# Urist-McDeveloper/nbody

Measured on AMD Instinct MI355X. Metric: particle-pair interactions/sec at N=2^20, higher is better.
Workload: dtype f32

## Files before the change

nbody_amd/csrc/kernels.h:

```cpp
#pragma once

#include <hip/hip_runtime.h>
#include <stdint.h>

namespace nb {

enum : uint32_t {
    STEP_ACC_IN = 1u,
    STEP_NO_FINALIZE = 2u,
};

enum : int {
    VARIANT_LDS = 0,
    VARIANT_SMEM = 1,
};

struct StepParams {
    const float2 *src_pos;
    const float *src_gm;
    uint32_t src_begin[2];
    uint32_t src_end[2];
    const float2 *pos_in;
    float2 *pos_out;
    float2 *vel;
    float2 *acc;
    const float *radius;
    uint32_t n_recv;
    uint32_t recv_split;
    uint32_t recv_gap;
    float2 *mirror;
    uint32_t n_mirror;
    const float *dt;
    uint32_t flags;
    float2 *parts;
    uint32_t split;
    uint32_t *tickets;
    uint32_t unit;
};

__host__ __device__ inline StepParams plain_step(const float2 *src_pos, const float *src_gm, uint32_t n_src, const float2 *pos_in,
                                                 float2 *pos_out, float2 *vel, float2 *acc, const float *radius, uint32_t n_recv,
                                                 const float *dt, uint32_t unit) {
    return StepParams{.src_pos = src_pos, .src_gm = src_gm, .src_begin = {0, 0}, .src_end = {n_src, 0}, .pos_in = pos_in,
                      .pos_out = pos_out, .vel = vel, .acc = acc, .radius = radius, .n_recv = n_recv, .recv_split = n_recv,
                      .dt = dt, .split = 1, .unit = unit};
}

struct ChainParams {
    float2 *pos;
    float2 *vel;
    float2 *acc;
// ... 34 lines not shown
};

struct RaggedParams {
    BatchParams b;
    const uint32_t *n_len;
    const uint32_t *members;
};

struct RaggedTraceParams {
    BatchTraceParams t;
    const uint32_t *n_len;
    const uint32_t *members;
};

constexpr int MAX_SPLIT = 16;

struct LaunchShape;

const void *step_kernel_fn(LaunchShape s);
const void *step_kernel_fused_fn(LaunchShape s);
const void *finish_kernel_fn();

void launch_chain(hipStream_t st, const ChainParams &p);

const void *batch_lane_split_fn(int w, int lanes);
void launch_batch_chain(hipStream_t st, const BatchParams &p, uint32_t count);
void launch_batch_trace_chain(hipStream_t st, const BatchTraceParams &p);

const void *ragged_lane_split_fn(int w, int lanes);
void launch_ragged_chain(hipStream_t st, const RaggedParams &p, uint32_t members);
void launch_ragged_trace_chain(hipStream_t st, const RaggedTraceParams &p, uint32_t members);

}
```

nbody_amd/csrc/kernels.hip:

```cpp
#include "kernels.h"
#include "diag_common.h"
#include "interaction_asm.h"
#include "launch_shape.h"

#include <hip/hip_runtime.h>

namespace nb {
namespace {

constexpr int WAVE = 64;
constexpr int CHUNK = 64;
constexpr int CLOSE_EVERY = 4;

typedef float v16f __attribute__((ext_vector_type(16)));
typedef float v8f __attribute__((ext_vector_type(8)));
typedef float v4f __attribute__((ext_vector_type(4)));

typedef float f2v __attribute__((ext_vector_type(2)));

template <int K>
struct Receivers {
    f2v p[K];
    float r[K];
    f2v a[K];
    f2v s[K];
    f2v c[K];
    __device__ __forceinline__ void clear() {
#pragma unroll
        for (int k = 0; k < K; k++) a[k] = s[k] = c[k] = f2v{0.0f, 0.0f};
    }
    __device__ __forceinline__ void close_chunk() {
#pragma unroll
        for (int k = 0; k < K; k++) {
            const f2v y = a[k] - c[k];
            const f2v t = s[k] + y;
            const f2v cn = (t - s[k]) - y;
            const bool lx = a[k].x != 0.0f, ly = a[k].y != 0.0f;
            const bool fx = __builtin_fabsf(t.x) < __builtin_inff(), fy = __builtin_fabsf(t.y) < __builtin_inff();
            c[k].x = lx ? (fx ? cn.x : 0.0f) : c[k].x;
            c[k].y = ly ? (fy ? cn.y : 0.0f) : c[k].y;
            s[k].x = lx ? t.x : s[k].x;
            s[k].y = ly ? t.y : s[k].y;
            a[k] = f2v{0.0f, 0.0f};
        }
    }
};


#define NB_INTERACT2(SRC)                                                                                                       \
    asm(NB_INTERACTION2_ASM                                                                                                     \
        : [ax0] "+v"(R.a[0].x), [ay0] "+v"(R.a[0].y), [ax1] "+v"(R.a[1].x), [ay1] "+v"(R.a[1].y)                                \
        : [sx] SRC(sxy.x), [sy] SRC(sxy.y), [g] SRC(sg), [px0] "v"(R.p[0].x), [py0] "v"(R.p[0].y), [r0] "v"(R.r[0]),            \
          [px1] "v"(R.p[1].x), [py1] "v"(R.p[1].y), [r1] "v"(R.r[1])                                                            \
        : NB_CLOBBERS2)
#define NB_INTERACT1(SRC)                                                                                                       \
    asm(NB_INTERACTION_ASM                                                                                                      \
        : [ax] "+v"(R.a[k].x), [ay] "+v"(R.a[k].y)                                                                              \
        : [sx] SRC(sxy.x), [sy] SRC(sxy.y), [g] SRC(sg), [px] "v"(R.p[k].x), [py] "v"(R.p[k].y), [r] "v"(R.r[k])                \
        : NB_CLOBBERS)
template <int K, bool SRC_IN_SGPR>
// ... 107 lines not shown
    const uint32_t logical = blockIdx.x * blockDim.x + threadIdx.x;
    if (logical >= p.n_recv) return;
    const uint32_t i = receiver_slot(p, logical);
    float2 part[MAX_SPLIT];
#pragma unroll
    for (uint32_t s = 0; s < (uint32_t)MAX_SPLIT; s++)
        part[s] = p.parts[(size_t)(s < p.split ? s : p.split - 1) * p.n_recv + logical];
    const float2 a0 = p.acc[i];
    const float2 v0 = p.vel[i];
    const float2 q0 = p.pos_in[i];
    const float dt = *p.dt;
    float sx = 0.0f, sy = 0.0f;
#pragma unroll
    for (uint32_t s = 0; s < (uint32_t)MAX_SPLIT; s++) add_part(sx, sy, part[s], s < p.split);
    finish_loaded(p, i, make_float2(sx, sy), a0, v0, q0, dt);
}

template <int K, int W, int VARIANT, bool FUSED = false>
__global__ __launch_bounds__(WAVE *W, 8) void step_kernel(const StepParams p) {
    const uint32_t tid = threadIdx.x;
    const uint32_t lane = tid & (WAVE - 1);
    const uint32_t wid = __builtin_amdgcn_readfirstlane(tid >> 6);
    const uint32_t tile_x = blockIdx.x, part_y = blockIdx.y;

    __shared__ __attribute__((aligned(16))) float tile[VARIANT == VARIANT_LDS ? W : 1][2][3 * CHUNK];
    __shared__ float2 partial[W > 1 ? W : 1][W > 1 ? WAVE * K : 1];

    const float dt = *p.dt;

    const uint32_t recv_base = tile_x * (WAVE * K);
// ... 36 lines not shown
            if (c + 1 < c_hi) fetch(c + 1);
            __builtin_amdgcn_fence(__ATOMIC_RELEASE, "wavefront");
            __builtin_amdgcn_wave_barrier();
            __builtin_amdgcn_fence(__ATOMIC_ACQUIRE, "wavefront");
            for (int jj = 0; jj < CHUNK; jj += 4) {
                const v8f P = *reinterpret_cast<const v8f *>(&T[buf][2 * jj]);
                const v4f G = *reinterpret_cast<const v4f *>(&T[buf][2 * CHUNK + jj]);
#pragma unroll
                for (int u = 0; u < 4; u++) interact<K, false>(R, f2v{P[2 * u], P[2 * u + 1]}, G[u]);
            }
            if (((c - c_lo) & (CLOSE_EVERY - 1)) == CLOSE_EVERY - 1) R.close_chunk();
            buf ^= 1;
        }
        if ((c_hi - c_lo) & (CLOSE_EVERY - 1)) R.close_chunk();
    } else {
#pragma unroll
        for (int range = 0; range < 2; range++) {
            const uint32_t r_lo = range == 0 ? 0u : n0;
            const uint32_t r_hi = range == 0 ? n0 : total;
            const uint32_t a = max(v_lo, r_lo), b = min(v_hi, r_hi);
            if (a >= b) continue;
            uint32_t j = p.src_begin[range] + (a - r_lo);
            const uint32_t j_end = p.src_begin[range] + (b - r_lo);
            const float *sp = reinterpret_cast<const float *>(p.src_pos), *sg = p.src_gm;
            const uint32_t groups = (j_end - j) / 8;
            const uint32_t g0 = (a - v_lo) / 8;
            if (groups > 0) {
                const uint32_t j_last = j + (groups - 1) * 8;
                v16f PA = src_load<v16f>(sp + 2 * (size_t)j);
                v8f GA = src_load<v8f>(sg + j);
                uint32_t g = 0;
                while (g + 2 <= groups) {
                    const uint32_t to_close = (8u * CLOSE_EVERY - ((g0 + g) & (8u * CLOSE_EVERY - 1))) / 2;
                    const uint32_t pairs = min(to_close, (groups - g) / 2);
                    for (uint32_t i = 0; i < pairs; i++) {
                        asm("" : "+s"(j) : "s"(PA), "s"(GA));
                        const v16f PB = src_load<v16f>(sp + 2 * (size_t)(j + 8));
                        const v8f GB = src_load<v8f>(sg + j + 8);
                        __builtin_amdgcn_sched_barrier(0);
                        interact8<K, true>(R, PA, GA);
                        __builtin_amdgcn_sched_barrier(0);
                        j = min(j + 16, j_last);
                        asm("" : "+s"(j) : "s"(PB), "s"(GB));
                        PA = src_load<v16f>(sp + 2 * (size_t)j);
                        GA = src_load<v8f>(sg + j);
                        __builtin_amdgcn_sched_barrier(0);
                        interact8<K, true>(R, PB, GB);
                    }
                    g += 2 * pairs;
                    if (pairs == to_close) R.close_chunk();
                }
                if (g < groups) interact8<K, true>(R, PA, GA);
                j = j_last + 8;
            }
            for (; j < j_end; j++) interact<K, true>(R, f2v{sp[2 * (size_t)j], sp[2 * (size_t)j + 1]}, sg[j]);
        }
        if ((v_hi - v_lo) & (CHUNK * CLOSE_EVERY - 1)) R.close_chunk();
    }

    auto finish = [&](uint32_t logical, float sx, float sy) {
        if (p.split > 1) {
            if (logical < p.n_recv) {
                float2 *slot = &p.parts[(size_t)part_y * p.n_recv + logical];
                if constexpr (FUSED) {
                    const uint64_t bits = (uint64_t)__float_as_uint(sx) | ((uint64_t)__float_as_uint(sy) << 32);
                    __hip_atomic_store(reinterpret_cast<uint64_t *>(slot), bits, __ATOMIC_RELAXED, __HIP_MEMORY_SCOPE_AGENT);
                } else {
                    *slot = make_float2(sx, sy);
                }
            }
        } else {
            finish_receiver(p, logical, sx, sy, dt);
        }
    };
// ... 32 lines not shown
                    for (uint32_t s = 0; s < (uint32_t)MAX_SPLIT; s++) {
                        const uint64_t bits = __hip_atomic_load(reinterpret_cast<const uint64_t *>(&p.parts[(size_t)(s < p.split ? s : p.split - 1) * p.n_recv + logical]),
                                                                __ATOMIC_RELAXED, __HIP_MEMORY_SCOPE_AGENT);
                        part[s] = make_float2(__uint_as_float((uint32_t)bits), __uint_as_float((uint32_t)(bits >> 32)));
                    }
                    const uint32_t i = receiver_slot(p, logical);
                    const float2 a0 = p.acc[i], v0 = p.vel[i], q0 = p.pos_in[i];
                    float sx = 0.0f, sy = 0.0f;
#pragma unroll
                    for (uint32_t s = 0; s < (uint32_t)MAX_SPLIT; s++) add_part(sx, sy, part[s], s < p.split);
                    finish_loaded(p, i, make_float2(sx, sy), a0, v0, q0, dt);
                }
            }
        }
    }
}

template <int W, int H>
__device__ __forceinline__ void lane_split_body(const StepParams &p) {
    constexpr uint32_t R = WAVE / H;
    constexpr uint32_t V = W * H;
    constexpr uint32_t T = 2 * WAVE * W;
    extern __shared__ __attribute__((aligned(16))) unsigned char lds_raw[];
    float2 *sxy = reinterpret_cast<float2 *>(lds_raw);
    float *sgm = reinterpret_cast<float *>(sxy + T);
    float2 *partial = reinterpret_cast<float2 *>(sgm + T);
    const uint32_t n0 = p.src_end[0] - p.src_begin[0];
    const uint32_t ntiles = (n0 + T - 1) / T;

    const uint32_t tid = threadIdx.x;
// ... 371 lines not shown

}

const void *step_kernel_fn(LaunchShape s) {
    if (s.lanes > 1) return pick_lane_split(s.w, s.lanes);
    return s.variant == VARIANT_SMEM ? pick<VARIANT_SMEM>(s.k, s.w) : pick<VARIANT_LDS>(s.k, s.w);
}

const void *step_kernel_fused_fn(LaunchShape s) {
    if (s.lanes > 1 || s.variant != VARIANT_SMEM) return nullptr;
    return pick_fused(s.k, s.w);
}

const void *finish_kernel_fn() { return reinterpret_cast<const void *>(&finish_kernel); }

const void *batch_lane_split_fn(int a, int b) {
    NB_CASE(batch_lane_split_kernel, 8, 8) NB_CASE(batch_lane_split_kernel, 16, 4)
    return nullptr;
}

const void *ragged_lane_split_fn(int a, int b) {
    NB_CASE(ragged_lane_split_kernel, 8, 8) NB_CASE(ragged_lane_split_kernel, 16, 4)
    return nullptr;
}
#undef NB_CASE

void launch_chain(hipStream_t st, const ChainParams &p) {
    hipLaunchKernelGGL(chain_kernel, dim3(1), dim3(1024), 0, st, p);
}

// ... 18 lines not shown
```

nbody_amd/csrc/launch_shape.h:

```cpp
#pragma once

#include "kernels.h"

namespace nb {

constexpr uint32_t BATCH_MAX_RECV = 3000;

struct LaunchShape {
    int k = 0;
    int w = 0;
    int variant = VARIANT_SMEM;
    int split = 0;
    int unit = 0;
    int lanes = 0;
};

inline bool operator==(const LaunchShape &a, const LaunchShape &b) {
    return a.k == b.k && a.w == b.w && a.variant == b.variant && a.split == b.split && a.unit == b.unit && a.lanes == b.lanes;
}

inline bool shape_on_auto(const LaunchShape &want) { return want == LaunchShape{}; }

constexpr uint32_t LANE_SPLIT_MAX_SRC = 1u << 18;

int lane_split_rule(uint32_t n_recv, uint32_t n_src, int *w);

LaunchShape choose_shape(LaunchShape want, uint32_t n_recv, uint32_t n_src, int compute_units);

bool fused_finish_rule(uint32_t n_recv, uint32_t n_src);

dim3 step_grid(LaunchShape s, uint32_t n_recv);
dim3 step_block(LaunchShape s);
size_t step_lds_bytes(LaunchShape s, uint32_t n_src);
dim3 finish_grid(uint32_t n_recv);
dim3 finish_block();

uint32_t chain_tiles(uint32_t n_recv);

int batch_lane_shape(uint32_t n_recv, int *w);

}
```

nbody_amd/csrc/launch_shape.hip:

```cpp
#include "launch_shape.h"

namespace nb {
namespace {

constexpr int WAVE = 64;
constexpr int CHUNK = 64;

double small_launch_cost_us(uint32_t n_recv, uint32_t n_src, int k, int w, int sp, int unit, int cus) {
    constexpr double LAT = 1.575, THR = 0.7545, K1 = 0.987, K1A = 0.178, A = 0.179, MIX = 0.874;
    constexpr double FINISH = 2.08, W4 = 1.035, UFIX = 0.15, BASE = 2.27;
    const uint32_t granules = (n_src + unit - 1) / unit;
    const uint64_t groups = ((uint64_t)n_recv + WAVE * k - 1) / (WAVE * k) * (uint64_t)sp;
    const uint64_t capacity = (uint64_t)cus * (32 / w);
    const uint64_t full = groups / capacity, left = groups % capacity;
    const uint32_t part_granules = (granules + sp - 1) / sp;
    const uint32_t wave_granules = (part_granules + w - 1) / w;
    const double units = (double)k * (wave_granules ? wave_granules : 1) * (double)unit / (double)CHUNK + UFIX;
    auto chunk_time = [&](double occ) {
        const double f = k == 1 ? K1 + K1A * (8.0 - occ) / 8.0 : 1.0;
        const double busy = occ * THR * f * (1.0 + A * (8.0 - occ) / 8.0);
        return LAT > busy ? LAT : busy;
    };
    double t = (double)full * units * chunk_time(8.0);
    if (left) {
// ... 116 lines not shown
uint32_t chain_tiles(uint32_t n_recv) {
    for (uint32_t t = 1; t <= 4; t *= 2)
        if (n_recv <= t * WAVE * CHAIN_K) return t;
    return 0;
}

int batch_lane_shape(uint32_t n_recv, int *w) { return lane_split_rule(n_recv, n_recv, w); }

constexpr double FUSED_FINISH_MIN_PAIRS = 4.0e7;
constexpr uint32_t FUSED_FINISH_MAX_RECV = 200000;

bool fused_finish_rule(uint32_t n_recv, uint32_t n_src) {
    return (double)n_recv * (double)n_src >= FUSED_FINISH_MIN_PAIRS && n_recv <= FUSED_FINISH_MAX_RECV;
}

}
```

nbody_amd/csrc/pipeline.hip:

```cpp
#include "pipeline_internal.h"
#include "nbody_hip_tuning.h"
#include "timestep.h"

using namespace nbi;

namespace {

void unpin_host(SimPipeline *s) {
    if (s->host_pinned) {
        (void)hipHostUnregister(s->host_array);
        s->host_pinned = false;
        s->host_dev = nullptr;
        s->host_current = false;
    }
}

void pin_host(SimPipeline *s) {
    if (s->host_pinned || s->host_array == nullptr || s->host_bytes == 0) return;
    if (hipHostRegister(s->host_array, s->host_bytes, hipHostRegisterMapped | hipHostRegisterPortable) == hipSuccess) {
        s->host_pinned = true;
        if (hipHostGetDevicePointer(&s->host_dev, s->host_array, 0) != hipSuccess) {
            (void)hipGetLastError();
            s->host_dev = nullptr;
        }
// ... 37 lines not shown
    dev_free(s->src_gm);
    dev_free(s->dt_dev);
    s->dt_dev = nullptr;
    s->dt_valid = false;
    dev_free(s->aos);
    dev_free(s->aos_shard);
    if (s->stage) ASSERT_HIP(hipHostFree(s->stage), "hipHostFree staging");
    s->stage = nullptr;
    s->stage_bytes = 0;
    dev_free(s->parts);
    s->parts = nullptr;
    s->parts_cap = 0;
    dev_free(s->tickets);
    s->tickets = nullptr;
    s->tickets_len = 0;
    dev_free(s->diag);
    s->diag = nullptr;
    s->diag_cap = 0;
    dev_free(s->diag_phi);
    s->diag_phi = nullptr;
    s->diag_phi_cap = 0;
    for (auto &e : s->ev_diag) {
        if (e) ASSERT_HIP(hipEventDestroy(e), "event");
        e = nullptr;
    }
    s->diag_timed = false;
    render_release(s);
    field_release(s);
    dev_free(s->adapt);
    s->adapt = nullptr;
// ... 104 lines not shown

extern "C" {

SimPipeline *CreateSimPipeline(WorldData data) {
    NB_ASSERT(data.mass_len <= data.total_len, "mass_len %u > total_len %u", data.mass_len, data.total_len);
    SimPipeline *s = new SimPipeline();
    s->data = data;
    s->plan = nb_hip_shard_plan(data.total_len, data.mass_len, 0, 1);
    const char *v = getenv("NB_HIP_VARIANT");
    if (v) s->want.variant = atoi(v) ? nb::VARIANT_SMEM : nb::VARIANT_LDS;
    const char *gr = getenv("NB_HIP_GRAPH");
    if (gr) s->use_graph = atoi(gr) < 0 || atoi(gr) > 2 ? 2 : atoi(gr);
#ifdef NB_TUNING_SHAPES
    struct { const char *env, *key; } presets[] = {
        {"NB_HIP_K", "k"}, {"NB_HIP_W", "w"}, {"NB_HIP_SPLIT", "split"}, {"NB_HIP_UNIT", "unit"}, {"NB_HIP_PASSES", "passes"},
        {"NB_HIP_LANES", "lanes"}, {"NB_HIP_FUSED_CHAIN", "fused_chain"}, {"NB_HIP_FUSED_FINISH", "fused_finish"},
        {"NB_HIP_READBACK", "readback"}, {"NB_HIP_ZERO_COPY_UPLOAD", "zero_copy_upload"},
    };
    for (const auto &p : presets)
        if (const char *e = getenv(p.env)) nb_hip_tune(s, p.key, atoi(e));
    if (const char *tm = getenv("NB_HIP_TIMING")) s->timing = atoi(tm) ? 1 : 0;
#endif
    return s;
}

SimPipeline *CreateSimPipelineSharded(WorldData data, int rank, int nranks, const void *unique_id128) {
    NB_ASSERT(nranks >= 1 && rank >= 0 && rank < nranks, "rank %d of %d", rank, nranks);
    const char *force = getenv("NB_HIP_FORCE_SHARDED");
    if (nranks == 1 && !(force && atoi(force))) return CreateSimPipeline(data);
    NB_ASSERT(unique_id128 != nullptr, "sharded pipeline needs the RCCL unique id");
    SimPipeline *s = CreateSimPipeline(data);
// ... 440 lines not shown
        old = s->want.lanes;
        s->want.lanes = value;
    } else if (!strcmp(key, "fused_chain")) {
        NB_ASSERT(value >= 0 && value <= 2, "fused_chain must be 0 (never), 1 (whenever the world fits one workgroup) or 2 (auto), got %d", value);
        old = s->fused_chain;
        s->fused_chain = value;
    } else if (!strcmp(key, "fused_finish")) {
        NB_ASSERT(value >= 0 && value <= 2, "fused_finish must be 0 (never), 1 (whenever the shape allows) or 2 (auto), got %d", value);
        old = s->fused_finish;
        if (s->on_device && old != value) {
            ASSERT_HIP(hipStreamSynchronize(s->stream), "sync before switching the finish mode");
            for (auto &g : s->graphs) destroy_graph(g);
            s->graphs.clear();
        }
        s->fused_finish = value;
    } else if (!strcmp(key, "passes")) {
        NB_ASSERT(value >= 0 && value <= 64, "passes must be 0 (auto) .. 64, got %d", value);
        old = s->want_passes;
        s->want_passes = value;
    } else if (!strcmp(key, "readback")) {
        NB_ASSERT(value >= 0 && value <= 2, "readback must be 0 (lazy), 1 (eager) or 2 (auto), got %d", value);
        old = s->readback;
        s->readback = value;
        s->frame_streak = 0;
    } else if (!strcmp(key, "render_merge")) {
        NB_ASSERT(value == 0 || value == 1, "render_merge must be 0 (one atomic per lane) or 1 (merged), got %d", value);
        old = s->render_merge;
        s->render_merge = value;
    } else if (!strcmp(key, "field_shape")) {
        NB_ASSERT(value >= 0 && value <= 2, "field_shape must be 0 (auto), 1 (source split) or 2 (one wave per tile), got %d", value);
// ... 29 lines not shown
```

nbody_amd/csrc/pipeline_internal.h:

```cpp
#pragma once

#include <hip/hip_runtime.h>

#include <stdint.h>
#include <stdio.h>
#include <stdlib.h>
#include <string.h>

#include <condition_variable>
#include <mutex>
#include <thread>
#include <utility>
#include <vector>

#include "convert.h"
#include "kernels.h"
#include "launch_shape.h"
#include "nbody_hip.h"


#define NB_FAIL(...)                                                          \
    do {                                                                      \
        fprintf(stderr, "%s:%d [%s] ", __FILE__, __LINE__, __func__);         \
        fprintf(stderr, __VA_ARGS__);                                         \
// ... 155 lines not shown
    void *aos_shard = nullptr;
    void *host_array = nullptr;
    size_t host_bytes = 0;
    bool host_pinned = false;
    void *host_dev = nullptr;
    int readback = 2;
    int zero_copy_upload = 1;
    bool host_current = false;
    uint32_t updates_since_get = 0, frame_streak = 0;
    int timing = 0;
    float2 *parts = nullptr;
    uint32_t parts_cap = 0;
    uint32_t *tickets = nullptr;
    uint32_t tickets_len = 0;
    int fused_finish = 2;
    int cur = 0;

    hipStream_t stream = nullptr;
    hipStream_t comm_stream = nullptr;
    hipEvent_t ev_begin = nullptr, ev_end = nullptr;
    hipEvent_t ev_local = nullptr, ev_gather = nullptr;
    bool timed = false;
    uint32_t timed_launches = 0;
    uint32_t timed_finish_launches = 0;
    nbi::EventPool pool;
    std::vector<std::pair<hipEvent_t, hipEvent_t>> kernel_iv, comm_iv;
    uint32_t detail_steps = 0;
    uint64_t use_clock = 0;

    nb::LaunchShape want;
// ... 79 lines not shown
```

nbody_amd/csrc/step_chain.hip:

```cpp
#include "pipeline_internal.h"
#include "timestep.h"
#include "timestep_common.h"

namespace nbi {

hipEvent_t EventPool::next() {
    if (used == ev.size()) {
        hipEvent_t e;
        ASSERT_HIP(hipEventCreate(&e), "event");
        ev.push_back(e);
    }
    return ev[used++];
}

void EventPool::destroy() {
    for (hipEvent_t e : ev) ASSERT_HIP(hipEventDestroy(e), "event");
    ev.clear();
    used = 0;
}

constexpr uint32_t GRAPH_CHAIN_MAX = 64;
constexpr size_t GRAPH_CACHE_MAX = 8;
constexpr uint32_t GRAPH_AUTO_MIN_CHAIN = 16;


void evict_for_one_more(SimPipeline *s) {
    while (s->graphs.size() >= GRAPH_CACHE_MAX) {
        size_t victim = 0;
        for (size_t i = 1; i < s->graphs.size(); i++)
            if (s->graphs[i].last_use < s->graphs[victim].last_use) victim = i;
        ASSERT_HIP(hipStreamSynchronize(s->stream), "sync before evicting a cached chain");
        destroy_graph(s->graphs[victim]);
        s->graphs.erase(s->graphs.begin() + (long)victim);
    }
}

uint32_t passes_for(const SimPipeline *s, const nb::StepParams &p);

void destroy_graph(StepGraph &g) {
    if (g.exec) ASSERT_HIP(hipGraphExecDestroy(g.exec), "hipGraphExecDestroy");
    if (g.graph) ASSERT_HIP(hipGraphDestroy(g.graph), "hipGraphDestroy");
    g.exec = nullptr;
    g.graph = nullptr;
    g.nodes.clear();
    g.params.clear();
}

nb::LaunchShape resolve_shape(SimPipeline *s) {
    nb::LaunchShape want = s->want;
    nb::StepParams probe;
    memset(&probe, 0, sizeof probe);
    probe.src_end[0] = s->n_src;
// ... 6 lines not shown
        if (need > s->parts_cap) {
            ASSERT_HIP(hipStreamSynchronize(s->stream), "sync before growing the parts buffer");
            dev_free(s->parts);
            s->parts = dev_alloc<float2>(need);
            s->parts_cap = (uint32_t)need;
            if (!s->tickets) {
                s->tickets_len = (uint32_t)((size_t)s->n_real / 64 + 2);
                s->tickets = dev_alloc<uint32_t>(s->tickets_len);
                zero_tickets(s);
                ASSERT_HIP(hipStreamSynchronize(s->stream), "sync after zeroing the tickets");
            }
            for (auto &g : s->graphs) destroy_graph(g);
            s->graphs.clear();
        }
    }
    s->last_shape = sh;
    s->last_groups = nb::step_grid(sh, s->n_real).x * nb::step_grid(sh, s->n_real).y;
    return sh;
}

nb::StepParams whole_step(const SimPipeline *s, int in, float dt) {
    (void)dt;
    nb::StepParams p = nb::plain_step(s->src_pos[in], s->src_gm, s->n_src, s->pos[in], s->pos[in ^ 1], s->vel, s->acc, s->radius,
                                      s->n_real, s->dt_dev, 64);
    if (s->sharded) {
        p.recv_split = s->plan.mass_count;
        p.recv_gap = s->plan.mass_chunk - s->plan.mass_count;
        p.mirror = s->src_pos[in ^ 1] + (size_t)s->rank * s->plan.mass_chunk;
        p.n_mirror = s->plan.mass_count;
    }
    return p;
}

bool fused_finish_applies(const SimPipeline *s, nb::LaunchShape sh) {
    if (s->fused_finish == 0 || s->sharded || sh.split <= 1 || sh.lanes > 1 || s->tickets == nullptr) return false;
    if (nb::step_kernel_fused_fn(sh) == nullptr) return false;
    return s->fused_finish == 1 || nb::fused_finish_rule(s->n_real, s->n_src);
}

nb::StepParams shaped(const SimPipeline *s, nb::StepParams p, nb::LaunchShape sh) {
    p.split = sh.split > 1 ? (uint32_t)sh.split : 1u;
    p.parts = p.split > 1 ? s->parts : nullptr;
    p.tickets = s->tickets;
    p.unit = (sh.unit >= 8 && sh.unit <= 64 && p.src_end[1] == p.src_begin[1]) ? (uint32_t)sh.unit : 64u;
    return p;
}

constexpr size_t L2_SOURCE_BUDGET = 3u << 20;

uint32_t passes_for(const SimPipeline *s, const nb::StepParams &p) {
    if (p.flags != 0 || p.src_end[1] != p.src_begin[1]) return 1;
    const uint32_t n = p.src_end[0] - p.src_begin[0];
    uint32_t want = (uint32_t)s->want_passes;
    if (want == 0) want = (uint32_t)(((size_t)n * 12 + L2_SOURCE_BUDGET - 1) / L2_SOURCE_BUDGET);
    const uint32_t chunks = (n + 63) / 64;
    if (want > chunks) want = chunks;
    return want ? want : 1;
}
// ... 5 lines not shown
    const uint32_t per = ((n + 63) / 64 + P - 1) / P * 64;
    for (uint32_t q = 0; q < P; q++) {
        nb::StepParams p = shaped(s, whole, sh);
        if (P > 1) {
            p.src_begin[0] = lo + (q * per < n ? q * per : n);
            p.src_end[0] = lo + ((q + 1) * per < n ? (q + 1) * per : n);
            p.flags = (q > 0 ? nb::STEP_ACC_IN : 0u) | (q + 1 < P ? nb::STEP_NO_FINALIZE : 0u);
        }
        out.push_back(p);
    }
    return out;
}

void launch_step(SimPipeline *s, nb::LaunchShape sh, const nb::StepParams &p, hipStream_t st) {
    if (s->n_real == 0) return;
    const bool fused = fused_finish_applies(s, sh);
    for (nb::StepParams &copy : step_passes(s, p, sh)) {
        void *args[] = {&copy};
        ASSERT_HIP(hipLaunchKernel(fused ? nb::step_kernel_fused_fn(sh) : nb::step_kernel_fn(sh), nb::step_grid(sh, s->n_real), nb::step_block(sh), args,
                                   nb::step_lds_bytes(sh, copy.src_end[0] - copy.src_begin[0]), st),
                   "step kernel launch (k=%d w=%d variant=%d split=%d, %u receivers)", sh.k, sh.w, sh.variant, sh.split,
                   s->n_real);
        if (copy.split > 1 && !fused)
            ASSERT_HIP(hipLaunchKernel(nb::finish_kernel_fn(), nb::finish_grid(s->n_real), nb::finish_block(), args, 0, st),
                       "finish kernel launch (%u receivers, %u parts)", s->n_real, copy.split);
    }
}

void zero_tickets(SimPipeline *s) {
    if (s->tickets && s->tickets_len)
        ASSERT_HIP(hipMemsetAsync(s->tickets, 0, (size_t)s->tickets_len * sizeof(uint32_t), s->stream), "zero the tile tickets");
}

void upload_dt(SimPipeline *s, float dt) {
    if (s->dt_valid && memcmp(&dt, &s->dt_enqueued, sizeof dt) == 0) return;
    nb::launch_set_scalar(s->stream, s->dt_dev, dt);
    s->dt_enqueued = dt;
    s->dt_valid = true;
    s->dt_uploads++;
// ... 8 lines not shown
    kp.sharedMemBytes = (unsigned int)lds_bytes;
    kp.kernelParams = args;
    kp.extra = nullptr;
}

StepGraph *find_graph(SimPipeline *s, uint32_t n, uint32_t passes, nb::LaunchShape sh, int phase) {
    for (auto &c : s->graphs)
        if (c.n == n && c.passes == passes && c.phase == phase && c.shape == sh) return &c;
    return nullptr;
}

StepGraph *find_or_build_graph(SimPipeline *s, uint32_t n, float dt, nb::LaunchShape sh) {
    const uint32_t passes = passes_for(s, whole_step(s, s->cur, dt));
    StepGraph *g = find_graph(s, n, passes, sh, s->cur);
    const bool fused = fused_finish_applies(s, sh);
    const uint32_t per_pass = sh.split > 1 && !fused ? 2 : 1;
    const uint32_t per_step = passes * per_pass;
    const bool fresh = g == nullptr;
    if (fresh) {
        evict_for_one_more(s);
        s->graphs.emplace_back();
        g = &s->graphs.back();
        g->n = n;
        g->passes = passes;
        g->shape = sh;
        ASSERT_HIP(hipGraphCreate(&g->graph, 0), "hipGraphCreate");
        g->nodes.resize((size_t)n * per_step);
        g->params.resize((size_t)n * passes);
    }
    g->last_use = ++s->use_clock;
    if (!fresh) return g;
    if (fused) zero_tickets(s);
    hipGraphNode_t prev = nullptr;
    for (uint32_t i = 0; i < n; i++) {
        const std::vector<nb::StepParams> launches = step_passes(s, whole_step(s, (s->cur + i) & 1, dt), sh);
        for (uint32_t q = 0; q < passes; q++) {
            g->params[(size_t)i * passes + q] = launches[q];
            void *args[] = {&g->params[(size_t)i * passes + q]};
            for (uint32_t j = 0; j < per_pass; j++) {
                hipKernelNodeParams kp;
                if (j == 0)
                    fill_node(kp, args, fused ? nb::step_kernel_fused_fn(sh) : nb::step_kernel_fn(sh), nb::step_grid(sh, s->n_real), nb::step_block(sh),
                              nb::step_lds_bytes(sh, launches[q].src_end[0] - launches[q].src_begin[0]));
                else
                    fill_node(kp, args, nb::finish_kernel_fn(), nb::finish_grid(s->n_real), nb::finish_block());
                hipGraphNode_t &node = g->nodes[(size_t)i * per_step + q * per_pass + j];
                ASSERT_HIP(hipGraphAddKernelNode(&node, g->graph, prev ? &prev : nullptr, prev ? 1 : 0, &kp),
                           "hipGraphAddKernelNode step %u/%u", i, n);
                prev = node;
            }
        }
    }
    ASSERT_HIP(hipGraphInstantiate(&g->exec, g->graph, nullptr, nullptr, 0), "hipGraphInstantiate (%u steps)", n);
    g->phase = s->cur;
    return g;
}

constexpr double CANON_MAX_PAIRS = 6.0e7;

constexpr double CHAIN_MAX_PAIRS = 3.6e4;
// ... 270 lines not shown
    s->kernel_iv.clear();
    s->comm_iv.clear();
    s->detail_steps = 0;
    s->fused_steps = 0;
    s->host_current = false;
    upload_dt(s, dt);
    if (s->timing) ASSERT_HIP(hipEventRecord(s->ev_begin, s->stream), "record begin");
    if (!s->sharded)
        enqueue_single(s, n, dt);
    else
        enqueue_sharded(s, n, dt);
    if (s->timing) ASSERT_HIP(hipEventRecord(s->ev_end, s->stream), "record end");
    s->timed = s->timing != 0;
    s->timed_launches = (s->sharded && s->overlap) ? 2 * n : n * passes_for(s, whole_step(s, s->cur, dt));
    if (s->fused_steps) s->timed_launches = (n + CHAIN_MAX_STEPS_PER_LAUNCH - 1) / CHAIN_MAX_STEPS_PER_LAUNCH;
    s->timed_finish_launches = s->last_shape.split > 1 && !fused_finish_applies(s, s->last_shape) ? s->timed_launches : 0;
    s->data.dt = dt;
}


void check_adaptive(const SimPipeline *s, uint32_t n, const NbAdaptive *cfg, const char *what) {
    NB_ASSERT(s != nullptr && cfg != nullptr, "%s: NULL argument", what);
    const char *fault = nb_timestep_cfg_fault(cfg);
    NB_ASSERT(fault == nullptr, "%s: %s (eta %g, dt_min %g, dt_max %g, span %g)", what, fault, (double)cfg->eta, (double)cfg->dt_min,
              (double)cfg->dt_max, cfg->span);
    NB_ASSERT(n <= NB_ADAPT_MAX_STEPS, "%s: %u steps > 2^20 in one call", what, n);
    NB_ASSERT(!s->sharded, "%s of a sharded pipeline needs a collective over the ranks: not supported", what);
    NB_ASSERT(n == 0 || s->on_device, "%s before SetSimulationData", what);
}

namespace {
// ... 49 lines not shown
        upload_dt(s, 0.0f);
        launch_step(s, sh, whole_step(s, s->cur, 0.0f), s->stream);
        s->cur ^= 1;
    }
    if (s->timing) ASSERT_HIP(hipEventRecord(s->ev_begin, s->stream), "record begin");
    for (uint32_t i = 0; i < n; i++) {
        p.log = log + i;
        nb::launch_timestep(s->stream, p);
        launch_step(s, sh, whole_step(s, s->cur, 0.0f), s->stream);
        s->cur ^= 1;
    }
    ASSERT_HIP(hipGetLastError(), "adaptive step launches (%u steps, %u particles)", n, s->n_real);
    if (s->timing) ASSERT_HIP(hipEventRecord(s->ev_end, s->stream), "record end");
    s->timed = s->timing != 0;
    s->timed_launches = n * passes_for(s, whole_step(s, s->cur, 0.0f));
    s->timed_finish_launches = s->last_shape.split > 1 && !fused_finish_applies(s, s->last_shape) ? s->timed_launches : 0;
    s->dt_valid = false;
    s->adapt_logged = n;
}

void enqueue_timestep_peek(SimPipeline *s, const NbAdaptive *cfg) {
    use_device();
    grow_adapt(s, 0);
    char *head = static_cast<char *>(s->adapt);
    nb::TimestepParams p = timestep_params(s, cfg);
    p.state = reinterpret_cast<nb::AdaptState *>(head + sizeof(nb::AdaptState));
    p.dt_out = reinterpret_cast<float *>(head + 2 * sizeof(nb::AdaptState));
    p.commit = 0;
    nb::launch_arm(s->stream, p.state, 1);
    nb::launch_timestep(s->stream, p);
    ASSERT_HIP(hipGetLastError(), "timestep_kernel launch (%u particles)", s->n_real);
// ... 4 lines not shown
```

Measured before the change: 5676 billion.

## Add opt-in slice-wave step form and hand-scheduled Kahan close for K=2

Adds a new step form where each 64-lane wave handles one source slice of a receiver tile and writes its partial sums to a slices buffer. A separate finish kernel then reduces the slices, which removes the in-block LDS cross-wave reduction. It also replaces the K=2 compensated-sum close with inline asm that takes a fast path when all accumulators are nonzero and finite. The slice form is off by default (slice_form=0), so only the asm close changes the default path, at the cost of extra code and a little branching per close.

```diff
diff --git a/nbody_amd/csrc/kernels.h b/nbody_amd/csrc/kernels.h
--- a/nbody_amd/csrc/kernels.h
+++ b/nbody_amd/csrc/kernels.h
@@ -35,6 +35,7 @@
     float2 *parts;
     uint32_t split;
     uint32_t *tickets;
+    float2 *slices;
     uint32_t unit;
 };
 
@@ -99,12 +100,15 @@
 };
 
 constexpr int MAX_SPLIT = 16;
+constexpr uint32_t SLICE_FORM_W = 16;
 
 struct LaunchShape;
 
 const void *step_kernel_fn(LaunchShape s);
 const void *step_kernel_fused_fn(LaunchShape s);
 const void *finish_kernel_fn();
+const void *slice_wave_kernel_fn(LaunchShape s);
+const void *slice_finish_kernel_fn();
 
 void launch_chain(hipStream_t st, const ChainParams &p);
 
diff --git a/nbody_amd/csrc/kernels.hip b/nbody_amd/csrc/kernels.hip
--- a/nbody_amd/csrc/kernels.hip
+++ b/nbody_amd/csrc/kernels.hip
@@ -22,28 +22,97 @@
 struct Receivers {
     f2v p[K];
     float r[K];
-    f2v a[K];
-    f2v s[K];
-    f2v c[K];
+    struct Sum {
+        float x, y;
+    };
+    Sum a[K];
+    Sum s[K];
+    Sum c[K];
     __device__ __forceinline__ void clear() {
 #pragma unroll
-        for (int k = 0; k < K; k++) a[k] = s[k] = c[k] = f2v{0.0f, 0.0f};
+        for (int k = 0; k < K; k++) a[k] = s[k] = c[k] = Sum{0.0f, 0.0f};
     }
     __device__ __forceinline__ void close_chunk() {
+        if constexpr (K == 2) {
+            close_pair();
+            return;
+        }
 #pragma unroll
         for (int k = 0; k < K; k++) {
-            const f2v y = a[k] - c[k];
-            const f2v t = s[k] + y;
-            const f2v cn = (t - s[k]) - y;
+            const float yx = __fsub_rn(a[k].x, c[k].x), yy = __fsub_rn(a[k].y, c[k].y);
+            const float tx = __fadd_rn(s[k].x, yx), ty = __fadd_rn(s[k].y, yy);
+            const float cnx = __fsub_rn(__fsub_rn(tx, s[k].x), yx), cny = __fsub_rn(__fsub_rn(ty, s[k].y), yy);
             const bool lx = a[k].x != 0.0f, ly = a[k].y != 0.0f;
-            const bool fx = __builtin_fabsf(t.x) < __builtin_inff(), fy = __builtin_fabsf(t.y) < __builtin_inff();
-            c[k].x = lx ? (fx ? cn.x : 0.0f) : c[k].x;
-            c[k].y = ly ? (fy ? cn.y : 0.0f) : c[k].y;
-            s[k].x = lx ? t.x : s[k].x;
-            s[k].y = ly ? t.y : s[k].y;
-            a[k] = f2v{0.0f, 0.0f};
-        }
-    }
+            const bool fx = __builtin_fabsf(tx) < __builtin_inff(), fy = __builtin_fabsf(ty) < __builtin_inff();
+            c[k].x = lx ? (fx ? cnx : 0.0f) : c[k].x;
+            c[k].y = ly ? (fy ? cny : 0.0f) : c[k].y;
+            s[k].x = lx ? tx : s[k].x;
+            s[k].y = ly ? ty : s[k].y;
+            a[k] = Sum{0.0f, 0.0f};
+        }
+    }
+#define NB_CLOSE_SELECT(A, S, C, T, Y)                                                                                          \
+    "v_sub_f32 %[d], %[" T "], %[" S "]\n\t"                                                                                    \
+    "v_sub_f32 %[d], %[d], %[" Y "]\n\t"                                                                                        \
+    "v_cmp_class_f32 vcc, %[" T "], %[finite]\n\t"                                                                              \
+    "s_nop 1\n\t"                                                                                                               \
+    "v_cndmask_b32 %[d], 0, %[d], vcc\n\t"                                                                                      \
+    "v_cmp_neq_f32 vcc, 0, %[" A "]\n\t"                                                                                        \
+    "s_nop 1\n\t"                                                                                                               \
+    "v_cndmask_b32 %[" C "], %[" C "], %[d], vcc\n\t"                                                                           \
+    "v_cndmask_b32 %[" S "], %[" S "], %[" T "], vcc\n\t"
+    __device__ __forceinline__ void close_pair() {
+        float y0, y1, y2, y3, t0, t1, t2, t3, z, d;
+        uint64_t mask;
+        asm("v_sub_f32 %[y0], %[a0], %[c0]\n\t"
+            "v_sub_f32 %[y1], %[a1], %[c1]\n\t"
+            "v_sub_f32 %[y2], %[a2], %[c2]\n\t"
+            "v_sub_f32 %[y3], %[a3], %[c3]\n\t"
+            "v_mul_f32 %[z], %[a0], %[a1]\n\t"
+            "v_add_f32 %[t0], %[s0], %[y0]\n\t"
+            "v_add_f32 %[t1], %[s1], %[y1]\n\t"
+            "v_add_f32 %[t2], %[s2], %[y2]\n\t"
+            "v_add_f32 %[t3], %[s3], %[y3]\n\t"
+            "v_mul_f32 %[z], %[z], %[a2]\n\t"
+            "v_add_f32 %[d], %[t0], %[t1]\n\t"
+            "v_mul_f32 %[z], %[z], %[a3]\n\t"
+            "v_add_f32 %[d], %[d], %[t2]\n\t"
+            "v_add_f32 %[d], %[d], %[t3]\n\t"
+            "v_cmp_nlt_f32_e64 vcc, 0, |%[z]|\n\t"
+            "v_cmp_class_f32 %[mask], %[d], %[nonfinite]\n\t"
+            "s_or_b64 vcc, vcc, %[mask]\n\t"
+            "s_cbranch_vccz .Lnb_close_plain_%=\n\t"
+            NB_CLOSE_SELECT("a0", "s0", "c0", "t0", "y0")
+            NB_CLOSE_SELECT("a1", "s1", "c1", "t1", "y1")
+            NB_CLOSE_SELECT("a2", "s2", "c2", "t2", "y2")
+            NB_CLOSE_SELECT("a3", "s3", "c3", "t3", "y3")
+            "s_branch .Lnb_close_done_%=\n"
+            ".Lnb_close_plain_%=:\n\t"
+            "v_sub_f32 %[c0], %[t0], %[s0]\n\t"
+            "v_sub_f32 %[c1], %[t1], %[s1]\n\t"
+            "v_sub_f32 %[c2], %[t2], %[s2]\n\t"
+            "v_sub_f32 %[c3], %[t3], %[s3]\n\t"
+            "v_sub_f32 %[c0], %[c0], %[y0]\n\t"
+            "v_sub_f32 %[c1], %[c1], %[y1]\n\t"
+            "v_sub_f32 %[c2], %[c2], %[y2]\n\t"
+            "v_sub_f32 %[c3], %[c3], %[y3]\n\t"
+            "v_mov_b32 %[s0], %[t0]\n\t"
+            "v_mov_b32 %[s1], %[t1]\n\t"
+            "v_mov_b32 %[s2], %[t2]\n\t"
+            "v_mov_b32 %[s3], %[t3]\n"
+            ".Lnb_close_done_%=:\n\t"
+            "v_mov_b32 %[a0], 0\n\t"
+            "v_mov_b32 %[a1], 0\n\t"
+            "v_mov_b32 %[a2], 0\n\t"
+            "v_mov_b32 %[a3], 0"
+            : [a0] "+v"(a[0].x), [a1] "+v"(a[0].y), [a2] "+v"(a[1].x), [a3] "+v"(a[1].y), [s0] "+v"(s[0].x), [s1] "+v"(s[0].y),
+              [s2] "+v"(s[1].x), [s3] "+v"(s[1].y), [c0] "+v"(c[0].x), [c1] "+v"(c[0].y), [c2] "+v"(c[1].x), [c3] "+v"(c[1].y),
+              [y0] "=&v"(y0), [y1] "=&v"(y1), [y2] "=&v"(y2), [y3] "=&v"(y3), [t0] "=&v"(t0), [t1] "=&v"(t1), [t2] "=&v"(t2),
+              [t3] "=&v"(t3), [z] "=&v"(z), [d] "=&v"(d), [mask] "=&s"(mask)
+            : [finite] "s"(0x1f8u), [nonfinite] "s"(0x207u)
+            : "vcc", "scc");
+    }
+#undef NB_CLOSE_SELECT
 };
 
 
@@ -181,6 +250,53 @@
 #pragma unroll
     for (uint32_t s = 0; s < (uint32_t)MAX_SPLIT; s++) add_part(sx, sy, part[s], s < p.split);
     finish_loaded(p, i, make_float2(sx, sy), a0, v0, q0, dt);
+}
+
+template <int K>
+__device__ __forceinline__ void walk_smem(Receivers<K> &R, const StepParams &p, uint32_t n0, uint32_t total, uint32_t v_lo,
+                                          uint32_t v_hi) {
+#pragma unroll
+    for (int range = 0; range < 2; range++) {
+        const uint32_t r_lo = range == 0 ? 0u : n0;
+        const uint32_t r_hi = range == 0 ? n0 : total;
+        const uint32_t a = max(v_lo, r_lo), b = min(v_hi, r_hi);
+        if (a >= b) continue;
+        uint32_t j = p.src_begin[range] + (a - r_lo);
+        const uint32_t j_end = p.src_begin[range] + (b - r_lo);
+        const float *sp = reinterpret_cast<const float *>(p.src_pos), *sg = p.src_gm;
+        const uint32_t groups = (j_end - j) / 8;
+        const uint32_t g0 = (a - v_lo) / 8;
+        if (groups > 0) {
+            const uint32_t j_last = j + (groups - 1) * 8;
+            v16f PA = src_load<v16f>(sp + 2 * (size_t)j);
+            v8f GA = src_load<v8f>(sg + j);
+            uint32_t g = 0;
+            while (g + 2 <= groups) {
+                const uint32_t to_close = (8u * CLOSE_EVERY - ((g0 + g) & (8u * CLOSE_EVERY - 1))) / 2;
+                const uint32_t pairs = min(to_close, (groups - g) / 2);
+                for (uint32_t i = 0; i < pairs; i++) {
+                    asm("" : "+s"(j) : "s"(PA), "s"(GA));
+                    const v16f PB = src_load<v16f>(sp + 2 * (size_t)(j + 8));
+                    const v8f GB = src_load<v8f>(sg + j + 8);
+                    __builtin_amdgcn_sched_barrier(0);
+                    interact8<K, true>(R, PA, GA);
+                    __builtin_amdgcn_sched_barrier(0);
+                    j = min(j + 16, j_last);
+                    asm("" : "+s"(j) : "s"(PB), "s"(GB));
+                    PA = src_load<v16f>(sp + 2 * (size_t)j);
+                    GA = src_load<v8f>(sg + j);
+                    __builtin_amdgcn_sched_barrier(0);
+                    interact8<K, true>(R, PB, GB);
+                }
+                g += 2 * pairs;
+                if (pairs == to_close) R.close_chunk();
+            }
+            if (g < groups) interact8<K, true>(R, PA, GA);
+            j = j_last + 8;
+        }
+        for (; j < j_end; j++) interact<K, true>(R, f2v{sp[2 * (size_t)j], sp[2 * (size_t)j + 1]}, sg[j]);
+    }
+    if ((v_hi - v_lo) & (CHUNK * CLOSE_EVERY - 1)) R.close_chunk();
 }
 
 template <int K, int W, int VARIANT, bool FUSED = false>
@@ -247,50 +363,11 @@
         }
         if ((c_hi - c_lo) & (CLOSE_EVERY - 1)) R.close_chunk();
     } else {
-#pragma unroll
-        for (int range = 0; range < 2; range++) {
-            const uint32_t r_lo = range == 0 ? 0u : n0;
-            const uint32_t r_hi = range == 0 ? n0 : total;
-            const uint32_t a = max(v_lo, r_lo), b = min(v_hi, r_hi);
-            if (a >= b) continue;
-            uint32_t j = p.src_begin[range] + (a - r_lo);
-            const uint32_t j_end = p.src_begin[range] + (b - r_lo);
-            const float *sp = reinterpret_cast<const float *>(p.src_pos), *sg = p.src_gm;
-            const uint32_t groups = (j_end - j) / 8;
-            const uint32_t g0 = (a - v_lo) / 8;
-            if (groups > 0) {
-                const uint32_t j_last = j + (groups - 1) * 8;
-                v16f PA = src_load<v16f>(sp + 2 * (size_t)j);
-                v8f GA = src_load<v8f>(sg + j);
-                uint32_t g = 0;
-                while (g + 2 <= groups) {
-                    const uint32_t to_close = (8u * CLOSE_EVERY - ((g0 + g) & (8u * CLOSE_EVERY - 1))) / 2;
-                    const uint32_t pairs = min(to_close, (groups - g) / 2);
-                    for (uint32_t i = 0; i < pairs; i++) {
-                        asm("" : "+s"(j) : "s"(PA), "s"(GA));
-                        const v16f PB = src_load<v16f>(sp + 2 * (size_t)(j + 8));
-                        const v8f GB = src_load<v8f>(sg + j + 8);
-                        __builtin_amdgcn_sched_barrier(0);
-                        interact8<K, true>(R, PA, GA);
-                        __builtin_amdgcn_sched_barrier(0);
-                        j = min(j + 16, j_last);
-                        asm("" : "+s"(j) : "s"(PB), "s"(GB));
-                        PA = src_load<v16f>(sp + 2 * (size_t)j);
-                        GA = src_load<v8f>(sg + j);
-                        __builtin_amdgcn_sched_barrier(0);
-                        interact8<K, true>(R, PB, GB);
-                    }
-                    g += 2 * pairs;
-                    if (pairs == to_close) R.close_chunk();
-                }
-                if (g < groups) interact8<K, true>(R, PA, GA);
-                j = j_last + 8;
-            }
-            for (; j < j_end; j++) interact<K, true>(R, f2v{sp[2 * (size_t)j], sp[2 * (size_t)j + 1]}, sg[j]);
-        }
-        if ((v_hi - v_lo) & (CHUNK * CLOSE_EVERY - 1)) R.close_chunk();
-    }
-
+        walk_smem<K>(R, p, n0, total, v_lo, v_hi);
+    }
+
+#pragma unroll
+    for (int k = 0; k < K; k++) asm("" : "+v"(R.s[k].x), "+v"(R.s[k].y));
     auto finish = [&](uint32_t logical, float sx, float sy) {
         if (p.split > 1) {
             if (logical < p.n_recv) {
@@ -353,6 +430,62 @@
             }
         }
     }
+}
+
+template <int K>
+__global__ __launch_bounds__(WAVE, 8) void slice_wave_kernel(const StepParams p) {
+    const uint32_t lane = threadIdx.x;
+    const uint32_t tile_x = blockIdx.x / SLICE_FORM_W, slice = blockIdx.x % SLICE_FORM_W, part_y = blockIdx.y;
+    const uint32_t recv_base = tile_x * (WAVE * K);
+    Receivers<K> R;
+#pragma unroll
+    for (int k = 0; k < K; k++) {
+        uint32_t i = recv_base + k * WAVE + lane;
+        i = i < p.n_recv ? i : p.n_recv - 1;
+        i = receiver_slot(p, i);
+        const float2 q = p.pos_in[i];
+        R.p[k] = f2v{q.x, q.y};
+        R.r[k] = p.radius[i];
+    }
+    R.clear();
+    const uint32_t n0 = p.src_end[0] - p.src_begin[0];
+    const uint32_t n1 = p.src_end[1] - p.src_begin[1];
+    const uint32_t total = n0 + n1;
+    const SourceSlice wave_src = source_slice(total, p.unit, p.split, part_y, SLICE_FORM_W, slice);
+    walk_smem<K>(R, p, n0, total, wave_src.lo, wave_src.hi);
+    float2 *out = p.slices + (size_t)(part_y * SLICE_FORM_W + slice) * p.n_recv;
+#pragma unroll
+    for (int k = 0; k < K; k++) asm("" : "+v"(R.s[k].x), "+v"(R.s[k].y));
+#pragma unroll
+    for (int k = 0; k < K; k++) {
+        const uint32_t logical = recv_base + k * WAVE + lane;
+        if (logical < p.n_recv) out[logical] = make_float2(R.s[k].x, R.s[k].y);
+    }
+}
+
+__global__ __launch_bounds__(256) void slice_finish_kernel(const StepParams p) {
+    const uint32_t logical = blockIdx.x * blockDim.x + threadIdx.x;
+    if (logical >= p.n_recv) return;
+    const uint32_t i = receiver_slot(p, logical);
+    const float2 a0 = p.acc[i];
+    const float2 v0 = p.vel[i];
+    const float2 q0 = p.pos_in[i];
+    const float dt = *p.dt;
+    float sx = 0.0f, sy = 0.0f;
+    for (uint32_t part = 0; part < p.split; part++) {
+        const float2 *first = p.slices + (size_t)part * SLICE_FORM_W * p.n_recv + logical;
+        float2 t[SLICE_FORM_W];
+#pragma unroll
+        for (uint32_t j = 0; j < SLICE_FORM_W; j++) t[j] = first[(size_t)j * p.n_recv];
+        float px = 0.0f, py = 0.0f;
+#pragma unroll
+        for (uint32_t j = 0; j < SLICE_FORM_W; j++) {
+            px = __fadd_rn(px, t[j].x);
+            py = __fadd_rn(py, t[j].y);
+        }
+        add_part(sx, sy, make_float2(px, py), true);
+    }
+    finish_loaded(p, i, make_float2(sx, sy), a0, v0, q0, dt);
 }
 
 template <int W, int H>
@@ -754,6 +887,15 @@
 
 const void *finish_kernel_fn() { return reinterpret_cast<const void *>(&finish_kernel); }
 
+const void *slice_wave_kernel_fn(LaunchShape s) {
+    if (s.lanes > 1 || s.variant != VARIANT_SMEM || s.w != (int)SLICE_FORM_W) return nullptr;
+    if (s.k == 1) return reinterpret_cast<const void *>(&slice_wave_kernel<1>);
+    if (s.k == 2) return reinterpret_cast<const void *>(&slice_wave_kernel<2>);
+    return nullptr;
+}
+
+const void *slice_finish_kernel_fn() { return reinterpret_cast<const void *>(&slice_finish_kernel); }
+
 const void *batch_lane_split_fn(int a, int b) {
     NB_CASE(batch_lane_split_kernel, 8, 8) NB_CASE(batch_lane_split_kernel, 16, 4)
     return nullptr;
diff --git a/nbody_amd/csrc/launch_shape.h b/nbody_amd/csrc/launch_shape.h
--- a/nbody_amd/csrc/launch_shape.h
+++ b/nbody_amd/csrc/launch_shape.h
@@ -29,6 +29,10 @@
 
 bool fused_finish_rule(uint32_t n_recv, uint32_t n_src);
 
+bool slice_form_rule(LaunchShape s, uint32_t n_recv, int compute_units);
+dim3 slice_grid(LaunchShape s, uint32_t n_recv);
+dim3 slice_block();
+
 dim3 step_grid(LaunchShape s, uint32_t n_recv);
 dim3 step_block(LaunchShape s);
 size_t step_lds_bytes(LaunchShape s, uint32_t n_src);
diff --git a/nbody_amd/csrc/launch_shape.hip b/nbody_amd/csrc/launch_shape.hip
--- a/nbody_amd/csrc/launch_shape.hip
+++ b/nbody_amd/csrc/launch_shape.hip
@@ -154,4 +154,17 @@
     return (double)n_recv * (double)n_src >= FUSED_FINISH_MIN_PAIRS && n_recv <= FUSED_FINISH_MAX_RECV;
 }
 
+constexpr uint64_t SLICE_FORM_MIN_ROUNDS = 4;
+
+bool slice_form_rule(LaunchShape s, uint32_t n_recv, int compute_units) {
+    if (compute_units <= 0) compute_units = 256;
+    const dim3 g = slice_grid(s, n_recv);
+    return (uint64_t)g.x * g.y >= SLICE_FORM_MIN_ROUNDS * 32u * (uint64_t)compute_units;
 }
+
+dim3 slice_grid(LaunchShape s, uint32_t n_recv) {
+    return dim3((n_recv + WAVE * s.k - 1) / (WAVE * s.k) * SLICE_FORM_W, s.split > 1 ? s.split : 1);
+}
+dim3 slice_block() { return dim3(WAVE); }
+
+}
diff --git a/nbody_amd/csrc/pipeline.hip b/nbody_amd/csrc/pipeline.hip
--- a/nbody_amd/csrc/pipeline.hip
+++ b/nbody_amd/csrc/pipeline.hip
@@ -75,6 +75,9 @@
     dev_free(s->tickets);
     s->tickets = nullptr;
     s->tickets_len = 0;
+    dev_free(s->slices);
+    s->slices = nullptr;
+    s->slices_cap = 0;
     dev_free(s->diag);
     s->diag = nullptr;
     s->diag_cap = 0;
@@ -209,7 +212,7 @@
 #ifdef NB_TUNING_SHAPES
     struct { const char *env, *key; } presets[] = {
         {"NB_HIP_K", "k"}, {"NB_HIP_W", "w"}, {"NB_HIP_SPLIT", "split"}, {"NB_HIP_UNIT", "unit"}, {"NB_HIP_PASSES", "passes"},
-        {"NB_HIP_LANES", "lanes"}, {"NB_HIP_FUSED_CHAIN", "fused_chain"}, {"NB_HIP_FUSED_FINISH", "fused_finish"},
+        {"NB_HIP_LANES", "lanes"}, {"NB_HIP_FUSED_CHAIN", "fused_chain"}, {"NB_HIP_FUSED_FINISH", "fused_finish"}, {"NB_HIP_SLICE_FORM", "slice_form"},
         {"NB_HIP_READBACK", "readback"}, {"NB_HIP_ZERO_COPY_UPLOAD", "zero_copy_upload"},
     };
     for (const auto &p : presets)
@@ -680,6 +683,15 @@
             s->graphs.clear();
         }
         s->fused_finish = value;
+    } else if (!strcmp(key, "slice_form")) {
+        NB_ASSERT(value >= 0 && value <= 2, "slice_form must be 0 (never), 1 (whenever the shape has the form) or 2 (auto), got %d", value);
+        old = s->slice_form;
+        if (s->on_device && old != value) {
+            ASSERT_HIP(hipStreamSynchronize(s->stream), "sync before switching the step form");
+            for (auto &g : s->graphs) destroy_graph(g);
+            s->graphs.clear();
+        }
+        s->slice_form = value;
     } else if (!strcmp(key, "passes")) {
         NB_ASSERT(value >= 0 && value <= 64, "passes must be 0 (auto) .. 64, got %d", value);
         old = s->want_passes;
diff --git a/nbody_amd/csrc/pipeline_internal.h b/nbody_amd/csrc/pipeline_internal.h
--- a/nbody_amd/csrc/pipeline_internal.h
+++ b/nbody_amd/csrc/pipeline_internal.h
@@ -193,6 +193,9 @@
     uint32_t *tickets = nullptr;
     uint32_t tickets_len = 0;
     int fused_finish = 2;
+    float2 *slices = nullptr;
+    size_t slices_cap = 0;
+    int slice_form = 0;
     int cur = 0;
 
     hipStream_t stream = nullptr;
diff --git a/nbody_amd/csrc/step_chain.hip b/nbody_amd/csrc/step_chain.hip
--- a/nbody_amd/csrc/step_chain.hip
+++ b/nbody_amd/csrc/step_chain.hip
@@ -36,6 +36,7 @@
 }
 
 uint32_t passes_for(const SimPipeline *s, const nb::StepParams &p);
+bool slice_form_applies(const SimPipeline *s, nb::LaunchShape sh);
 
 void destroy_graph(StepGraph &g) {
     if (g.exec) ASSERT_HIP(hipGraphExecDestroy(g.exec), "hipGraphExecDestroy");
@@ -72,6 +73,17 @@
             s->graphs.clear();
         }
     }
+    if (slice_form_applies(s, sh)) {
+        const size_t need = (size_t)nb::SLICE_FORM_W * (sh.split > 1 ? sh.split : 1) * s->n_real;
+        if (need > s->slices_cap) {
+            ASSERT_HIP(hipStreamSynchronize(s->stream), "sync before growing the slice sums");
+            dev_free(s->slices);
+            s->slices = dev_alloc<float2>(need);
+            s->slices_cap = need;
+            for (auto &g : s->graphs) destroy_graph(g);
+            s->graphs.clear();
+        }
+    }
     s->last_shape = sh;
     s->last_groups = nb::step_grid(sh, s->n_real).x * nb::step_grid(sh, s->n_real).y;
     return sh;
@@ -96,10 +108,29 @@
     return s->fused_finish == 1 || nb::fused_finish_rule(s->n_real, s->n_src);
 }
 
+bool slice_form_applies(const SimPipeline *s, nb::LaunchShape sh) {
+    if (s->slice_form == 0 || s->n_real == 0 || nb::slice_wave_kernel_fn(sh) == nullptr || fused_finish_applies(s, sh)) return false;
+    return s->slice_form == 1 || nb::slice_form_rule(sh, s->n_real, g_dev.compute_units);
+}
+
+struct PassKernels {
+    const void *step, *finish;
+    dim3 grid, block;
+};
+
+PassKernels pass_kernels(const SimPipeline *s, nb::LaunchShape sh) {
+    if (slice_form_applies(s, sh))
+        return {nb::slice_wave_kernel_fn(sh), nb::slice_finish_kernel_fn(), nb::slice_grid(sh, s->n_real), nb::slice_block()};
+    const bool fused = fused_finish_applies(s, sh);
+    return {fused ? nb::step_kernel_fused_fn(sh) : nb::step_kernel_fn(sh), sh.split > 1 && !fused ? nb::finish_kernel_fn() : nullptr,
+            nb::step_grid(sh, s->n_real), nb::step_block(sh)};
+}
+
 nb::StepParams shaped(const SimPipeline *s, nb::StepParams p, nb::LaunchShape sh) {
     p.split = sh.split > 1 ? (uint32_t)sh.split : 1u;
     p.parts = p.split > 1 ? s->parts : nullptr;
     p.tickets = s->tickets;
+    p.slices = s->slices;
     p.unit = (sh.unit >= 8 && sh.unit <= 64 && p.src_end[1] == p.src_begin[1]) ? (uint32_t)sh.unit : 64u;
     return p;
 }
@@ -135,15 +166,14 @@
 
 void launch_step(SimPipeline *s, nb::LaunchShape sh, const nb::StepParams &p, hipStream_t st) {
     if (s->n_real == 0) return;
-    const bool fused = fused_finish_applies(s, sh);
+    const PassKernels kn = pass_kernels(s, sh);
     for (nb::StepParams &copy : step_passes(s, p, sh)) {
         void *args[] = {&copy};
-        ASSERT_HIP(hipLaunchKernel(fused ? nb::step_kernel_fused_fn(sh) : nb::step_kernel_fn(sh), nb::step_grid(sh, s->n_real), nb::step_block(sh), args,
-                                   nb::step_lds_bytes(sh, copy.src_end[0] - copy.src_begin[0]), st),
+        ASSERT_HIP(hipLaunchKernel(kn.step, kn.grid, kn.block, args, nb::step_lds_bytes(sh, copy.src_end[0] - copy.src_begin[0]), st),
                    "step kernel launch (k=%d w=%d variant=%d split=%d, %u receivers)", sh.k, sh.w, sh.variant, sh.split,
                    s->n_real);
-        if (copy.split > 1 && !fused)
-            ASSERT_HIP(hipLaunchKernel(nb::finish_kernel_fn(), nb::finish_grid(s->n_real), nb::finish_block(), args, 0, st),
+        if (kn.finish)
+            ASSERT_HIP(hipLaunchKernel(kn.finish, nb::finish_grid(s->n_real), nb::finish_block(), args, 0, st),
                        "finish kernel launch (%u receivers, %u parts)", s->n_real, copy.split);
     }
 }
@@ -182,7 +212,8 @@
     const uint32_t passes = passes_for(s, whole_step(s, s->cur, dt));
     StepGraph *g = find_graph(s, n, passes, sh, s->cur);
     const bool fused = fused_finish_applies(s, sh);
-    const uint32_t per_pass = sh.split > 1 && !fused ? 2 : 1;
+    const PassKernels kn = pass_kernels(s, sh);
+    const uint32_t per_pass = kn.finish ? 2 : 1;
     const uint32_t per_step = passes * per_pass;
     const bool fresh = g == nullptr;
     if (fresh) {
@@ -208,10 +239,9 @@
             for (uint32_t j = 0; j < per_pass; j++) {
                 hipKernelNodeParams kp;
                 if (j == 0)
-                    fill_node(kp, args, fused ? nb::step_kernel_fused_fn(sh) : nb::step_kernel_fn(sh), nb::step_grid(sh, s->n_real), nb::step_block(sh),
-                              nb::step_lds_bytes(sh, launches[q].src_end[0] - launches[q].src_begin[0]));
+                    fill_node(kp, args, kn.step, kn.grid, kn.block, nb::step_lds_bytes(sh, launches[q].src_end[0] - launches[q].src_begin[0]));
                 else
-                    fill_node(kp, args, nb::finish_kernel_fn(), nb::finish_grid(s->n_real), nb::finish_block());
+                    fill_node(kp, args, kn.finish, nb::finish_grid(s->n_real), nb::finish_block());
                 hipGraphNode_t &node = g->nodes[(size_t)i * per_step + q * per_pass + j];
                 ASSERT_HIP(hipGraphAddKernelNode(&node, g->graph, prev ? &prev : nullptr, prev ? 1 : 0, &kp),
                            "hipGraphAddKernelNode step %u/%u", i, n);
@@ -512,7 +542,7 @@
     s->timed = s->timing != 0;
     s->timed_launches = (s->sharded && s->overlap) ? 2 * n : n * passes_for(s, whole_step(s, s->cur, dt));
     if (s->fused_steps) s->timed_launches = (n + CHAIN_MAX_STEPS_PER_LAUNCH - 1) / CHAIN_MAX_STEPS_PER_LAUNCH;
-    s->timed_finish_launches = s->last_shape.split > 1 && !fused_finish_applies(s, s->last_shape) ? s->timed_launches : 0;
+    s->timed_finish_launches = pass_kernels(s, s->last_shape).finish ? s->timed_launches : 0;
     s->data.dt = dt;
 }
 
@@ -592,7 +622,7 @@
     if (s->timing) ASSERT_HIP(hipEventRecord(s->ev_end, s->stream), "record end");
     s->timed = s->timing != 0;
     s->timed_launches = n * passes_for(s, whole_step(s, s->cur, 0.0f));
-    s->timed_finish_launches = s->last_shape.split > 1 && !fused_finish_applies(s, s->last_shape) ? s->timed_launches : 0;
+    s->timed_finish_launches = pass_kernels(s, s->last_shape).finish ? s->timed_launches : 0;
     s->dt_valid = false;
     s->adapt_logged = n;
 }
```

After: 5683 billion (median of 4 runs). No clear change (+0.1%).
